# nirajbabar/raytracinginonesemester

Measured on AMD Instinct MI355X. Metric: Mrays/s at 1920x1080x16spp (1/2/4/8 GPU) + PPM max-abs pixel diff, higher is better.
Workload: dtype f32+f64

## Files before the change

### include/rt_mi355x.h

```cpp
#ifndef RT_MI355X_H
#define RT_MI355X_H

#include <stddef.h>
#include <stdint.h>

#ifdef __cplusplus
extern "C" {
#endif

#define RT_ABI_VERSION 3

enum {
    RT_OK = 0,
    RT_ERR_ARG = -1,
    RT_ERR_IO = -2,
    RT_ERR_PARSE = -3,
    RT_ERR_HIP = -4,
    RT_ERR_NOMEM = -5,
    RT_ERR_NODEVICE = -6,
    RT_ERR_UNSUPPORTED = -7,
    RT_ERR_COMM = -8,
    RT_ERR_INTERNAL = -9
};

// ... 142 lines not shown
int rt_render(rt_scene* s, const rt_camera* cam, const rt_render_opts* opt,
              float* rgb_host, int32_t* hit_idx_host, float* hit_t_host);

int rt_count_rays(rt_scene* s, const rt_camera* cam, const rt_render_opts* opt, uint64_t counts[3]);
int rt_count_rays_ex(rt_scene* s, const rt_camera* cam, const rt_render_opts* opt, uint64_t counts[4]);

int rt_render_reference(size_t num_triangles, int W, int H, const rt_camera* cam, rt_vec3 miss_color,
                        int max_depth, int spp, const rt_bvh_node* nodes, const rt_aabb* aabbs,
                        const rt_triangle* triangles, const int32_t* tri_object_ids,
                        const rt_material* materials, int num_materials, const rt_light* lights,
                        int num_lights, int diffuse_bounce, rt_vec3* output);

int rt_render_reference_gpus(size_t num_triangles, int W, int H, const rt_camera* cam, rt_vec3 miss_color,
                             int max_depth, int spp, const rt_bvh_node* nodes, const rt_aabb* aabbs,
                             const rt_triangle* triangles, const int32_t* tri_object_ids,
                             const rt_material* materials, int num_materials, const rt_light* lights,
                             int num_lights, int diffuse_bounce, int n_gpus, rt_vec3* output);

typedef struct rt_renderer rt_renderer;

enum {
    RT_DELIVER_P6 = 0,
    RT_DELIVER_F32 = 1,
    RT_DELIVER_DEVICE = 2,
    RT_DELIVER_NONE = 3
};
enum {
    RT_GATHER_AUTO = 0,
    RT_GATHER_RCCL = 1,
    RT_GATHER_DIRECT = 2,
    RT_GATHER_HOST_SHARED = 3
};
enum { RT_RENDERER_SELF_SEND = 1  };

typedef struct {
    int32_t n_devices;
    const int32_t* devices;
    int32_t world_size;
    int32_t rank0;
    const void* unique_id;
    int32_t band_rows;
    int32_t deliver;
    int32_t gather;
    int32_t depth;
    int32_t flags;
    const char* host_frame_name;
} rt_renderer_opts;
void rt_renderer_opts_default(rt_renderer_opts* o);

int rt_renderer_copy_engine(const rt_renderer* r);

int rt_comm_unique_id(void* id128);

int rt_renderer_create(size_t num_triangles, const rt_bvh_node* nodes, const rt_aabb* aabbs,
                       const rt_triangle* triangles, const int32_t* tri_object_ids,
                       const rt_material* materials, int num_materials, const rt_light* lights,
                       int num_lights, const rt_renderer_opts* opts, rt_renderer** out);
void rt_renderer_destroy(rt_renderer* r);

int rt_renderer_submit(rt_renderer* r, const rt_camera* cam, const rt_render_opts* opts, uint64_t* ticket);
int rt_renderer_submit_pair(rt_renderer* r, const rt_camera* cam_a, const rt_camera* cam_b,
                            const rt_render_opts* opts, uint64_t* ticket_a);
int rt_renderer_wait(rt_renderer* r, uint64_t ticket, const void** frame, size_t* bytes);
int rt_renderer_render(rt_renderer* r, const rt_camera* cam, const rt_render_opts* opts, void* out, size_t cap);
rt_scene* rt_renderer_scene(rt_renderer* r, int i);
int rt_renderer_local_ranks(const rt_renderer* r);
enum { RT_TIME_GATHER = 0, RT_TIME_DELIVER = 1, RT_TIME_FRAME = 2  };
int rt_renderer_times(rt_renderer* r, int kind, float* ms_out, int max, int* n_out);

int rt_render_hw1(int device, const rt_vec3* positions, const rt_vec3* normals,
                  const uint32_t* indices, size_t num_triangles, const rt_camera* cam,
                  rt_vec3 light_position, rt_vec3 light_color, int spp, const float* jitter,
                  float* rgb_host, int32_t* hit_idx_host, float* hit_t_host);

enum { RT_HW1_BRUTE = 1 };
int rt_render_hw1_ex(int device, const rt_vec3* positions, const rt_vec3* normals,
                     const uint32_t* indices, size_t num_triangles, const rt_camera* cam,
                     rt_vec3 light_position, rt_vec3 light_color, int spp, const float* jitter,
                     int flags, float* rgb_host, int32_t* hit_idx_host, float* hit_t_host,
                     float* kernel_ms);

typedef struct rt_hw1_scene rt_hw1_scene;
int rt_hw1_scene_create(int device, const rt_vec3* positions, const rt_vec3* normals, const uint32_t* indices,
                        size_t num_triangles, rt_hw1_scene** out);
void rt_hw1_scene_destroy(rt_hw1_scene* s);
int rt_render_hw1_device(rt_hw1_scene* s, const rt_camera* cam, rt_vec3 light_position, rt_vec3 light_color,
                         int spp, const float* jitter, int flags, float* rgb_dev, uint8_t* p6_dev,
                         int32_t* hit_idx_dev, float* hit_t_dev, void* hip_stream);
int rt_render_hw1_deliver(rt_hw1_scene* s, const rt_camera* cam, rt_vec3 light_position, rt_vec3 light_color,
                          int spp, int flags, uint8_t* host_p6, void* hip_stream, uint64_t* ticket);
int rt_hw1_wait(rt_hw1_scene* s, uint64_t ticket);
int rt_hw1_kernel_times(const rt_hw1_scene* s, float* ms_out, int max, int* n_out);
const char* rt_hw1_kernel_name(const rt_hw1_scene* s);
int rt_hw1_list_info(const rt_hw1_scene* s, int64_t info[2]);

int rt_intersect_rays(int device, const rt_triangle* tri, const float origin[3], const float* dirs, int n,
                      int hw1, float tmin, float tmax, int32_t* hit, float* t);

typedef struct { rt_vec3 origin, direction; } rt_ray;
enum { RT_RAYS_CLOSEST = 0, RT_RAYS_OCCLUDED = 1 };
enum { RT_RAYS_VARIANT_NONE = 0, RT_RAYS_VARIANT_WIDE = 1, RT_RAYS_VARIANT_BINARY = 2, RT_RAYS_VARIANT_DEEP = 3 };

int rt_trace_rays_device(rt_scene* s, int mode, const rt_ray* rays_dev, const float* max_t_dev, size_t n,
                         int flags, int32_t* hit_idx_dev, float* hit_t_dev, void* hip_stream);
int rt_trace_rays(rt_scene* s, int mode, const rt_ray* rays, const float* max_t, size_t n, int flags,
                  int32_t* hit_idx, float* hit_t, float* kernel_ms);
int rt_trace_rays_variant(const rt_scene* s);

float rt_powf_host(float x, float y);
int rt_powf_batch(int device, const float* x, const float* y, int n, float* out);

int rt_box_test_host(const float* rays, const float* boxes, const float* tminmax, int n,
                     int32_t* out_fast, int32_t* out_exact, int32_t* out_class);

int rt_debug_frustum_records(size_t P, const rt_bvh_node* nodes, const rt_aabb* aabbs, int max_log2, int stack_cap,
                             int64_t* info, float* rec, size_t rec_cap);

int rt_kernel_times(const rt_scene* s, float* ms_out, int max, int* n_out);
int rt_frame_times(const rt_scene* s, float* ms_out, int max, int* n_out);
int rt_prepass_times(const rt_scene* s, float* ms_out, int max, int* n_out);
int rt_live_tiles(const rt_scene* s, int64_t* live, int64_t* total);
int rt_heavy_tiles(const rt_scene* s, int64_t* heavy);
const char* rt_scene_kernel_name(const rt_scene* s);

int rt_scene_traversal_info(const rt_scene* s, int64_t info[4]);
int rt_scene_faults(rt_scene* s, uint32_t* flags, int clear);

typedef enum {
    RT_TUNE_FRUSTUM_ARITY = 0,
    RT_TUNE_HALF_WAVES = 1,
    RT_TUNE_PAIRED_ONLY = 2,
    RT_TUNE_HEAVY_FRAC = 3,
    RT_TUNE_HEAVY_CAP = 4,
    RT_TUNE_CULL_COVERAGE = 5,
    RT_TUNE_CULL_BOXES = 6,
    RT_TUNE_BIG_SCENE_BYTES = 7,
    RT_TUNE_FRUSTUM_STACK_CAP = 8,
    RT_TUNE_PEER_TIMEOUT_S = 9,
    RT_TUNE_RENDERER_THREADS = 10,
    RT_TUNE_COPY_ENGINE = 11,
    RT_TUNE_QUANT_RECORDS = 12,
    RT_TUNE_PREPASS_GATE = 13,
    RT_TUNE_OVERLAP_FRAMES = 14,
    RT_TUNE_KERNEL_TIMING_EVERY = 15,
    RT_TUNE_RECORD_GREEDY = 16,
    RT_TUNE_WIDE4_GREEDY = 17,
    RT_TUNE_PAIR_FRAMES = 18,
    RT_TUNE_PAIR_RESERVE = 19,
    RT_TUNE_CUT_SUB = 20,
    RT_TUNE_HW1_LANES = 21,
    RT_TUNE_COPY_WAIT = 22,
    RT_TUNE_HW1_FUSE = 23,
    RT_TUNE_HW1_CHUNK = 24,
    RT_TUNE_COUNT = 25
} rt_tune_id;
int rt_tuning_set(int id, double value);
int rt_tuning_get(int id, double* value);
void rt_tuning_reset(void);

int rt_device_count(int* n);
const char* rt_last_error(void);
int rt_abi_version(void);
const char* rt_build_id(void);

#ifdef __cplusplus
}
#endif
#endif
```

### raytracinginonesemester_amd/_lib.py

```python
from __future__ import annotations

import ctypes as C
import os
from pathlib import Path

PKG = Path(__file__).resolve().parent
LIB_PATH = Path(os.environ.get("RT_MI355X_LIB", PKG / "lib" / "librt_mi355x.so"))

RT_OK = 0
RT_ERR = {
    -1: "RT_ERR_ARG", -2: "RT_ERR_IO", -3: "RT_ERR_PARSE", -4: "RT_ERR_HIP",
    -5: "RT_ERR_NOMEM", -6: "RT_ERR_NODEVICE", -7: "RT_ERR_UNSUPPORTED", -8: "RT_ERR_COMM",
    -9: "RT_ERR_INTERNAL",
}
RT_KERNEL_AUTO, RT_KERNEL_WAVE, RT_KERNEL_LANE, RT_KERNEL_WAVE_PIXELS = 0, 1, 2, 3
RT_TILES_AUTO, RT_TILES_LINEAR, RT_TILES_XCD_CHUNK, RT_TILES_ROWS = 0, 1, 2, 3
RT_FLAG_NO_CULL = 1
RT_FLAG_BINARY = 4
RT_DELIVER_P6, RT_DELIVER_F32, RT_DELIVER_DEVICE, RT_DELIVER_NONE = 0, 1, 2, 3
RT_GATHER_AUTO, RT_GATHER_RCCL, RT_GATHER_DIRECT, RT_GATHER_HOST_SHARED = 0, 1, 2, 3
RT_RENDERER_SELF_SEND = 1
RT_TIME_GATHER, RT_TIME_DELIVER, RT_TIME_FRAME = 0, 1, 2
RT_FAULT_FRUSTUM_STACK = 1
RT_RAYS_CLOSEST, RT_RAYS_OCCLUDED = 0, 1
RT_RAYS_VARIANT_NONE, RT_RAYS_VARIANT_WIDE, RT_RAYS_VARIANT_BINARY, RT_RAYS_VARIANT_DEEP = 0, 1, 2, 3
TUNE = {"frustum_arity": 0, "half_waves": 1, "paired_only": 2, "heavy_frac": 3, "heavy_cap": 4,
        "cull_coverage": 5, "cull_boxes": 6, "big_scene_bytes": 7, "frustum_stack_cap": 8,
        "peer_timeout_s": 9, "renderer_threads": 10, "copy_engine": 11,
        "quant_records": 12, "prepass_gate": 13,
        "overlap_frames": 14, "kernel_timing_every": 15,
        "record_greedy": 16, "wide4_greedy": 17, "pair_frames": 18, "pair_reserve": 19,
        "cut_sub": 20, "hw1_lanes": 21, "copy_wait": 22, "hw1_fuse": 23, "hw1_chunk": 24}


class RTError(RuntimeError):
    def __init__(self, code: int, msg: str):
        super().__init__(f"{RT_ERR.get(code, code)}: {msg}")
        self.code = code


class Vec3(C.Structure):
    _fields_ = [("x", C.c_float), ("y", C.c_float), ("z", C.c_float)]

    def __iter__(self):
        return iter((self.x, self.y, self.z))


class BVHNode(C.Structure):
    _fields_ = [("parent_idx", C.c_uint32), ("left_idx", C.c_uint32),
                ("right_idx", C.c_uint32), ("object_idx", C.c_uint32)]


class AABB(C.Structure):
    _fields_ = [("min_corner", Vec3), ("max_corner", Vec3)]


class Triangle(C.Structure):
    _fields_ = [("v0", Vec3), ("v1", Vec3), ("v2", Vec3), ("n0", Vec3), ("n1", Vec3), ("n2", Vec3)]


class Material(C.Structure):
    _fields_ = [("albedo", Vec3), ("kd", C.c_float), ("specular_color", Vec3), ("ks", C.c_float),
                ("shininess", C.c_float), ("kr", C.c_float), ("emission", Vec3)]


class Light(C.Structure):
    _fields_ = [("position", Vec3), ("color", Vec3), ("intensity", C.c_int32)]


class CameraT(C.Structure):
    _fields_ = [("center", Vec3), ("pixel00_loc", Vec3), ("pixel_delta_u", Vec3),
                ("pixel_delta_v", Vec3), ("pixel_width", C.c_int32), ("pixel_height", C.c_int32)]


class SceneInfo(C.Structure):
    _fields_ = [("max_depth", C.c_int32), ("spp", C.c_int32), ("diffuse_bounce", C.c_int32),
                ("miss_color", Vec3), ("cam_position", Vec3), ("cam_look_at", Vec3), ("cam_up", Vec3),
                ("focal_length_mm", C.c_double), ("sensor_height_mm", C.c_double),
                ("pixel_width", C.c_int32), ("pixel_height", C.c_int32),
                ("num_triangles", C.c_uint64), ("num_vertices", C.c_uint64),
                ("num_materials", C.c_int32), ("num_lights", C.c_int32),
                ("num_objects_loaded", C.c_int32), ("bvh_max_stack", C.c_int32),
                ("bvh_height", C.c_int32)]


class SceneArrays(C.Structure):
    _fields_ = [("nodes", C.c_void_p), ("aabbs", C.c_void_p), ("triangles", C.c_void_p),
                ("tri_object_ids", C.c_void_p), ("materials", C.c_void_p), ("lights", C.c_void_p),
                ("positions", C.c_void_p), ("normals", C.c_void_p), ("indices", C.c_void_p)]


class MeshView(C.Structure):
    _fields_ = [("positions", C.c_void_p), ("normals", C.c_void_p), ("indices", C.c_void_p),
                ("num_vertices", C.c_uint64), ("num_triangles", C.c_uint64),
                ("has_normals", C.c_int32), ("has_uvs", C.c_int32)]


class PPMOptions(C.Structure):
    _fields_ = [("maxval", C.c_int32), ("clamp", C.c_int32), ("gamma2", C.c_int32), ("flip_y", C.c_int32)]


class RenderOpts(C.Structure):
    _fields_ = [("max_depth", C.c_int32), ("spp", C.c_int32), ("diffuse_bounce", C.c_int32),
                ("miss_color", Vec3), ("jitter", C.c_void_p), ("band_rows", C.c_int32),
                ("band_index", C.c_int32), ("band_count", C.c_int32), ("kernel", C.c_int32),
                ("tile_order", C.c_int32), ("flags", C.c_int32)]


class RendererOpts(C.Structure):
    _fields_ = [("n_devices", C.c_int32), ("devices", C.c_void_p), ("world_size", C.c_int32),
                ("rank0", C.c_int32), ("unique_id", C.c_void_p), ("band_rows", C.c_int32),
                ("deliver", C.c_int32), ("gather", C.c_int32), ("depth", C.c_int32), ("flags", C.c_int32),
                ("host_frame_name", C.c_void_p)]


P = C.c_void_p
I = C.c_int
SZ = C.c_size_t

SIGNATURES = {
    "rt_material_default": (None, [P]),
    "rt_camera_init": (I, [P, P, P, P, C.c_double, C.c_double, I, I, I]),
    "rt_jittered_samples": (I, [I, C.c_uint32, I, P]),
    "rt_host_scene_load_json": (I, [C.c_char_p, C.c_char_p, P]),
    "rt_host_scene_load_objs": (I, [P, I, P]),
    "rt_host_scene_info": (I, [P, P]),
    "rt_host_scene_arrays": (I, [P, P]),
    "rt_host_scene_free": (None, [P]),
    "rt_build_bvh": (I, [P, SZ, P, SZ, P, P]),
    "rt_build_bvh_device": (I, [I, P, SZ, P, SZ, P, P, P]),
    "rt_mesh_load_obj_hw1": (I, [C.c_char_p, P]),
    "rt_mesh_view_get": (I, [P, P]),
    "rt_mesh_free": (None, [P]),
    "rt_ppm_options_default": (None, [P]),
    "rt_ppm_write": (I, [C.c_char_p, P, I, I, P]),
    "rt_ppm_encode": (I, [P, I, I, P, P, SZ, P]),
    "rt_ppm_read": (I, [C.c_char_p, P, SZ, P, P, P]),
    "rt_ppm_header": (I, [I, I, I, P, SZ, P]),
    "rt_ppm_quantize_device": (I, [P, I, I, P, P, P]),
    "rt_unpermute_strips_device": (I, [P, I, SZ, I, I, I, I, P, P]),
    "rt_scene_create": (I, [I, SZ, P, P, P, P, P, I, P, I, P]),
    "rt_scene_destroy": (None, [P]),
    "rt_scene_clone": (I, [P, I, P]),
    "rt_scene_device": (I, [P]),
    "rt_scene_device_bytes": (SZ, [P]),
    "rt_render_opts_default": (None, [P]),
    "rt_shard_rows": (I, [I, I, I, I]),
    "rt_render_device": (I, [P, P, P, P, P, P, P]),
    "rt_render_device_p6": (I, [P, P, P, P, P, P, P, P]),
    "rt_render_device_pair": (I, [P, P, P, P, P, P, P, P, P]),
    "rt_render": (I, [P, P, P, P, P, P]),
    "rt_count_rays": (I, [P, P, P, P]),
    "rt_count_rays_ex": (I, [P, P, P, P]),
    "rt_render_reference": (I, [SZ, I, I, P, Vec3, I, I, P, P, P, P, P, I, P, I, I, P]),
    "rt_render_reference_gpus": (I, [SZ, I, I, P, Vec3, I, I, P, P, P, P, P, I, P, I, I, I, P]),
    "rt_renderer_opts_default": (None, [P]),
    "rt_comm_unique_id": (I, [P]),
    "rt_renderer_create": (I, [SZ, P, P, P, P, P, I, P, I, P, P]),
    "rt_renderer_destroy": (None, [P]),
    "rt_renderer_submit": (I, [P, P, P, P]),
    "rt_renderer_submit_pair": (I, [P, P, P, P, P]),
    "rt_renderer_wait": (I, [P, C.c_uint64, P, P]),
    "rt_renderer_render": (I, [P, P, P, P, SZ]),
    "rt_renderer_scene": (P, [P, I]),
    "rt_renderer_local_ranks": (I, [P]),
    "rt_renderer_copy_engine": (I, [P]),
    "rt_renderer_times": (I, [P, I, P, I, P]),
    "rt_render_hw1": (I, [I, P, P, P, SZ, P, Vec3, Vec3, I, P, P, P, P]),
    "rt_render_hw1_ex": (I, [I, P, P, P, SZ, P, Vec3, Vec3, I, P, I, P, P, P, P]),
    "rt_hw1_scene_create": (I, [I, P, P, P, SZ, P]),
    "rt_hw1_scene_destroy": (None, [P]),
    "rt_render_hw1_device": (I, [P, P, Vec3, Vec3, I, P, I, P, P, P, P, P]),
    "rt_render_hw1_deliver": (I, [P, P, Vec3, Vec3, I, I, P, P, P]),
    "rt_hw1_wait": (I, [P, C.c_uint64]),
    "rt_hw1_kernel_times": (I, [P, P, I, P]),
    "rt_hw1_kernel_name": (C.c_char_p, [P]),
    "rt_hw1_list_info": (I, [P, P]),
    "rt_intersect_rays": (I, [I, P, P, P, I, I, C.c_float, C.c_float, P, P]),
    "rt_trace_rays_device": (I, [P, I, P, P, SZ, I, P, P, P]),
    "rt_trace_rays": (I, [P, I, P, P, SZ, I, P, P, P]),
    "rt_trace_rays_variant": (I, [P]),
    "rt_powf_host": (C.c_float, [C.c_float, C.c_float]),
    "rt_debug_frustum_records": (C.c_int, [C.c_size_t, P, P, C.c_int, C.c_int, P, P, C.c_size_t]),
    "rt_powf_batch": (I, [I, P, P, I, P]),
    "rt_box_test_host": (I, [P, P, P, I, P, P, P]),
# ... 53 lines not shown
```

### raytracinginonesemester_amd/csrc/rt_device.hip

```cpp

#include <hip/hip_runtime.h>
#include <hip/hip_ext.h>

#include <cfloat>
#include <cmath>
#include <cstdint>
#include <cstdio>
#include <cstdlib>
#include <cstring>
#include <algorithm>
#include <atomic>
#include <functional>
#include <memory>
#include <new>
#include <string>
#include <array>
#include <vector>

#include "rt_common.hpp"
#include "rt_hip_host.hpp"
#include "rt_math.hpp"
#include "rt_ppm.hpp"
#include "rt_records.hpp"

// ... 1017 lines not shown
        if (hipOccupancyMaxActiveBlocksPerMultiprocessor(&n, KERNEL, BLOCK, 0) != hipSuccess || n < 1) n = 1;
        return n;
    }();
    static const std::string name = "render_tiles_kernel<" + std::to_string(MODE) + (SAMPLES ? ", true" : ", false") +
                                    (D1 ? ", true, " : ", false, ") + std::to_string(WAVES) + ", " +
                                    std::to_string(LS) + ">";
    if (L.name) *L.name = name.c_str();
    const int tiles8 = (P.tiles_total + 7) / 8 * 8;
    const dim3 grid((unsigned)std::max(8, std::min(tiles8, L.cus * per_cu / 8 * 8)));
    hipExtLaunchKernelGGL(KERNEL, grid, dim3(BLOCK), 0, L.st, L.start, L.stop, 0, P);
}

template <int MODE, bool SAMPLES, bool D1, int WAVES = RT_RENDER_WAVES, int LS = 0>
void launch_render_pair(const RenderParams& A, const RenderParams& B, const Launch& L, double reserve_default) {
    constexpr auto KERNEL = render_pair_kernel<MODE, SAMPLES, D1, WAVES, LS>;
    static const int per_cu = [] {
        int n = 0;
        if (hipOccupancyMaxActiveBlocksPerMultiprocessor(&n, KERNEL, BLOCK, 0) != hipSuccess || n < 1) n = 1;
        return n;
    }();
    static const std::string name = "render_pair_kernel<" + std::to_string(MODE) + (SAMPLES ? ", true" : ", false") +
                                    (D1 ? ", true, " : ", false, ") + std::to_string(WAVES) + ", " +
                                    std::to_string(LS) + ">";
    if (L.name) *L.name = name.c_str();
    const int tiles8 = (A.tiles_total + B.tiles_total + 7) / 8 * 8;
    const double reserve = std::clamp(rt::tuning(RT_TUNE_PAIR_RESERVE, reserve_default), 0.0, double(per_cu - 1));
    const int blocks = L.cus * per_cu - int(std::lround(reserve * L.cus));
    const dim3 grid((unsigned)std::max(8, std::min(tiles8, blocks / 8 * 8)));
    PairParams PP;
    PP.f[0] = A;
    PP.f[1] = B;
    hipExtLaunchKernelGGL(KERNEL, grid, dim3(BLOCK), 0, L.st, L.start, L.stop, 0, PP);
}

bool pair_kernel_fits(const RenderParams& P, bool samples, bool wave_wide, bool big) {
    const bool d1 = P.max_depth == 1;
    const bool bounce = P.max_depth > 1 && P.half_waves && P.paired_only;
    return samples && wave_wide && !big && (d1 || bounce) && P.nqueues == 8 && P.spp <= 64 && !P.ray_count &&
           P.lane_samples == 1;
}
void launch_pair(const RenderParams& A, const RenderParams& B, const Launch& L) {
    constexpr int M = RT_KERNEL_WAVE | MODE_WIDE | MODE_PK;
    if (A.max_depth > 1) launch_render_pair<RT_KERNEL_WAVE | MODE_WIDE, true, false, RT_PAIRED_WAVES, 3>(A, B, L, 0.0);
    else if (A.half_waves) launch_render_pair<M, true, true, RT_RENDER_WAVES, 1>(A, B, L, 1.0);
    else launch_render_pair<M, true, true>(A, B, L, 1.0);
}

template <int MODE, bool SAMPLES>
void launch_mode(const RenderParams& P, const Launch& L) {
    constexpr int D1_MODE = (MODE & (MODE_DEEP | RT_KERNEL_LANE)) == 0 ? (MODE | MODE_PK) : MODE;
    if (P.max_depth == 1) {
        if constexpr (SAMPLES) {
            if (P.half_waves) {
                launch_render<D1_MODE, SAMPLES, true, RT_RENDER_WAVES, 1>(P, L);
                return;
            }
        }
        if constexpr ((MODE & (MODE_DEEP | RT_KERNEL_LANE)) == 0) {
            if (L.big) {
                if constexpr ((MODE & MODE_WIDE) != 0) {
                    if (L.qr) {
                        if (P.sc.num_lights == 1)
                            launch_render<D1_MODE | MODE_1L | MODE_QR, SAMPLES, true, RT_RENDER_WAVES_BIG>(P, L);
                        else launch_render<D1_MODE | MODE_QR, SAMPLES, true, RT_RENDER_WAVES_BIG>(P, L);
                        return;
                    }
                }
                if (P.sc.num_lights == 1) launch_render<D1_MODE | MODE_1L, SAMPLES, true, RT_RENDER_WAVES_BIG>(P, L);
                else launch_render<D1_MODE, SAMPLES, true, RT_RENDER_WAVES_BIG>(P, L);
                return;
            }
        }
        launch_render<D1_MODE, SAMPLES, true>(P, L);
    } else {
        if constexpr (SAMPLES && (MODE & (MODE_DEEP | RT_KERNEL_LANE)) == 0) {
            if (P.half_waves && P.paired_only) {
                launch_render<MODE, SAMPLES, false, RT_PAIRED_WAVES, 3>(P, L);
                return;
            }
        }
        if constexpr (SAMPLES) {
            if (P.half_waves) {
                launch_render<MODE, SAMPLES, false, RT_BOUNCE_WAVES, 1>(P, L);
                return;
            }
        }
        launch_render<MODE, SAMPLES, false, RT_BOUNCE_WAVES>(P, L);
    }
}

template <int MODE>
void launch(const RenderParams& P, bool samples, const Launch& L) {
    if (samples) launch_mode<MODE, true>(P, L);
    else launch_mode<MODE, false>(P, L);
}

f3 miss_pixel_value(const rt_render_opts* o) {
    f3 c = mk(0.f, 0.f, 0.f);
    if (o->max_depth > 0)
        c = clamp01(add(mk(0.f, 0.f, 0.f), mul(mk(1.f, 1.f, 1.f), f3{o->miss_color.x, o->miss_color.y, o->miss_color.z})));
    f3 acc = mk(0.f, 0.f, 0.f);
    for (int k = 0; k < o->spp; ++k) acc = add(acc, c);
    const float fs = (float)o->spp;
    return f3{acc.x / fs, acc.y / fs, acc.z / fs};
}

}

namespace {
double root_box_coverage(const float* rb, const rt_camera* cam) {
    const double c[3] = {cam->center.x, cam->center.y, cam->center.z};
    const double b0[3] = {cam->pixel00_loc.x - c[0], cam->pixel00_loc.y - c[1], cam->pixel00_loc.z - c[2]};
    const double du[3] = {cam->pixel_delta_u.x, cam->pixel_delta_u.y, cam->pixel_delta_u.z};
    const double dv[3] = {cam->pixel_delta_v.x, cam->pixel_delta_v.y, cam->pixel_delta_v.z};
    auto det3 = [](const double* x, const double* y, const double* z) {
        return x[0] * (y[1] * z[2] - y[2] * z[1]) - y[0] * (x[1] * z[2] - x[2] * z[1]) + z[0] * (x[1] * y[2] - x[2] * y[1]);
    };
    const double D = det3(b0, du, dv);
    if (!(std::fabs(D) > 0.0) || !(rb[0] <= rb[3] && rb[1] <= rb[4] && rb[2] <= rb[5])) return 1.0;
    double x0 = INFINITY, x1 = -INFINITY, y0 = INFINITY, y1 = -INFINITY;
    for (int k = 0; k < 8; ++k) {
        const double p[3] = {double(rb[(k & 1) ? 3 : 0]) - c[0], double(rb[(k & 2) ? 4 : 1]) - c[1],
                             double(rb[(k & 4) ? 5 : 2]) - c[2]};
        const double sx = det3(p, du, dv) / D, a = det3(b0, p, dv) / D, b = det3(b0, du, p) / D;
        if (!(sx > 0.0)) return 1.0;
        x0 = std::min(x0, a / sx);
        x1 = std::max(x1, a / sx);
        y0 = std::min(y0, b / sx);
        y1 = std::max(y1, b / sx);
    }
    const double W = cam->pixel_width, H = cam->pixel_height;
    const double w = std::max(0.0, std::min(W, x1) - std::max(0.0, x0)), h = std::max(0.0, std::min(H, y1) - std::max(0.0, y0));
    return w * h / (W * H);
}
}

thread_local unsigned long long* t_ray_count = nullptr;

extern "C" int rt_render_device(rt_scene* s, const rt_camera* cam, const rt_render_opts* o, float* rgb,
                                int32_t* hit_idx, float* hit_t, void* stream) {
    return rt_render_device_p6(s, cam, o, rgb, hit_idx, hit_t, nullptr, stream);
}

namespace {
struct PairStage {
    int phase = 0;
    bool deferred = false;
    RenderParams A;
    Launch LA{};
    uint64_t kA = 0;
    hipStream_t stream = nullptr;
};

int launch_prepasses(rt_scene* s, const RenderParams& P, int slot) {
    const bool cut = P.cull && P.sc.ncut > 0;
    hipExtLaunchKernelGGL(tile_cull_kernel, dim3((P.tiles_total + BLOCK - 1) / BLOCK), dim3(BLOCK), 0, s->prep,
                          s->ev0[slot], cut ? nullptr : s->pdone[slot], 0, P);
    HIP_TRY(hipGetLastError());
    if (cut) {
        const int cut_blocks = 4 * s->cus;
        hipExtLaunchKernelGGL(tile_cut_kernel, dim3(cut_blocks), dim3(BLOCK), 0, s->prep, nullptr, s->pdone[slot], 0, P);
        HIP_TRY(hipGetLastError());
    }
    return RT_OK;
}

int flush_pair_a(rt_scene* s, PairStage& ps) {
    if (!ps.deferred) return RT_OK;
    ps.deferred = false;
    const int slot = int(ps.kA % rt_scene::kRing);
    s->span[slot] = 1;
    if (int rc = launch_prepasses(s, ps.A, slot); rc != RT_OK) return rc;
    HIP_TRY(hipStreamWaitEvent(ps.LA.st, s->pdone[slot], 0));
    launch<RT_KERNEL_WAVE | MODE_WIDE>(ps.A, true, ps.LA);
    HIP_TRY(hipGetLastError());
    if (ps.A.drained) s->drain_frame = ps.kA;
    return RT_OK;
}

int render_frame(rt_scene* s, const rt_camera* cam, const rt_render_opts* o, float* rgb, int32_t* hit_idx,
                 float* hit_t, uint8_t* p6, void* stream, PairStage* ps);
}

extern "C" int rt_render_device_p6(rt_scene* s, const rt_camera* cam, const rt_render_opts* o, float* rgb,
                                   int32_t* hit_idx, float* hit_t, uint8_t* p6, void* stream) {
    return render_frame(s, cam, o, rgb, hit_idx, hit_t, p6, stream, nullptr);
}

extern "C" int rt_render_device_pair(rt_scene* s, const rt_camera* cam_a, const rt_camera* cam_b,
                                     const rt_render_opts* o, float* rgb_a, uint8_t* p6_a, float* rgb_b,
                                     uint8_t* p6_b, void* stream) {
    if (!s || !cam_a || !cam_b || !o || (!rgb_a && !p6_a) || (!rgb_b && !p6_b))
        return set_error(RT_ERR_ARG, "rt_render_device_pair: null argument");
    PairStage ps;
    int rc = render_frame(s, cam_a, o, rgb_a, nullptr, nullptr, p6_a, stream, &ps);
    if (rc != RT_OK) return rc;
    ps.phase = 1;
    rc = render_frame(s, cam_b, o, rgb_b, nullptr, nullptr, p6_b, stream, &ps);
    if (ps.deferred) {
        DeviceGuard g(s->device);
        const int rc2 = flush_pair_a(s, ps);
        if (rc == RT_OK) rc = rc2;
    }
    return rc;
}

namespace {
int render_frame(rt_scene* s, const rt_camera* cam, const rt_render_opts* o, float* rgb, int32_t* hit_idx,
                 float* hit_t, uint8_t* p6, void* stream, PairStage* ps) {
    if (!s || !cam || !o || (!rgb && !p6)) return set_error(RT_ERR_ARG, "rt_render_device: null argument");
    if (o->spp < 1) return set_error(RT_ERR_ARG, "spp must be >= 1");
    if ((hit_idx == nullptr) != (hit_t == nullptr)) return set_error(RT_ERR_ARG, "hit_idx and hit_t go together");
    const int W = cam->pixel_width, H = cam->pixel_height;
    if (W < 1 || H < 1) return set_error(RT_ERR_ARG, "camera has no pixels");
    const int rows = rt_shard_rows(H, o->band_rows, o->band_index, o->band_count);
    if (rows < 0) return set_error(RT_ERR_ARG, "bad band sharding parameters");
    DeviceGuard g(s->device);
    int rc = prepare_jitter(s, o);
    if (rc != RT_OK) return rc;
    if (rows == 0) return RT_OK;

    RenderParams P;
    std::memset(&P, 0, sizeof(P));
    P.sc.inode = static_cast<const float4*>(s->inode.p);
    P.sc.wnode = static_cast<const float4*>(s->wnode.p);
    P.sc.fnode = static_cast<const float*>(s->fnode.p);
    P.sc.f_log2 = s->fnode.p ? s->f_log2 : 2;
    P.sc.qent = static_cast<const uint4*>(s->qent.p);
    P.sc.qhdr = static_cast<const float4*>(s->qhdr.p);
    P.sc.wide = s->wide && !(o->flags & RT_FLAG_BINARY) ? 1 : 0;
    P.sc.lane_stack = s->lane_stack ? 1 : 0;
    P.sc.lane_wide = s->lane_wide ? 1 : 0;
    P.sc.ibox = static_cast<const float4*>(s->ibox.p);
    P.sc.rootb = static_cast<const float4*>(s->ibox.p) + s->ibox.n / sizeof(float4) - 2;
    P.sc.leaf = static_cast<const float4*>(s->leaf.p);
    P.sc.tnorm = static_cast<const float4*>(s->tnorm.p);
    P.sc.objids = static_cast<const int32_t*>(s->objids.p);
    P.sc.mats = static_cast<const DevMaterial*>(s->mats.p);
    P.sc.lights = static_cast<const DevLight*>(s->lights.p);
    P.sc.num_tris = int32_t(s->P);
    P.sc.num_mats = s->nmat;
    P.sc.num_lights = s->nlights;
    P.sc.root_ref = s->root_ref;
    std::memcpy(P.sc.root_box, s->root_box, sizeof(P.sc.root_box));
    P.sc.cut = static_cast<const float*>(s->cut.p);
    P.sc.cut2 = static_cast<const float*>(s->cut2.p);
    P.sc.cut_sub_log2 = s->cut2.p ? s->cut_sub_log2 : 0;
    P.sc.tri = static_cast<const float4*>(s->tri.p);
    P.sc.fault = static_cast<uint32_t*>(s->fault.p);
    const double max_cov = rt::tuning(RT_TUNE_CULL_COVERAGE, 0.3);
    P.sc.ncut = s->ncut > 0 && root_box_coverage(s->root_box, cam) <= max_cov ? s->ncut : 0;
    P.cut_force = max_cov >= 1.0 ? 1 : 0;
    std::memcpy(P.sc.bmax, s->bmax, sizeof(P.sc.bmax));
    P.cam_center = f3{cam->center.x, cam->center.y, cam->center.z};
    P.cam_p00 = f3{cam->pixel00_loc.x, cam->pixel00_loc.y, cam->pixel00_loc.z};
    P.cam_du = f3{cam->pixel_delta_u.x, cam->pixel_delta_u.y, cam->pixel_delta_u.z};
    P.cam_dv = f3{cam->pixel_delta_v.x, cam->pixel_delta_v.y, cam->pixel_delta_v.z};
    P.W = W;
    P.H = H;
    P.spp = o->spp;
    P.max_depth = o->max_depth;
    P.diffuse_bounce = o->diffuse_bounce ? 1 : 0;
    P.miss = f3{o->miss_color.x, o->miss_color.y, o->miss_color.z};
    P.jitter = static_cast<const float*>(s->jitter.p);
    P.band_rows = o->band_count <= 1 ? H : o->band_rows;
    P.band_index = o->band_count <= 1 ? 0 : o->band_index;
    P.band_count = o->band_count <= 1 ? 1 : o->band_count;
    P.rows = rows;
    P.rgb = rgb;
    P.hit_idx = hit_idx;
    P.hit_t = hit_t;
    P.p6 = p6;
    P.ray_count = t_ray_count;
    {
        const f3 mp = miss_pixel_value(o);
        P.miss_p6[0] = rtp::p6_default_sample(mp.x);
        P.miss_p6[1] = rtp::p6_default_sample(mp.y);
        P.miss_p6[2] = rtp::p6_default_sample(mp.z);
        P.miss_p6[3] = 0;
    }
    const bool samples = o->kernel != RT_KERNEL_WAVE_PIXELS && o->spp <= BLOCK && (o->spp & (o->spp - 1)) == 0;
    int half = o->band_count >= 4 || o->max_depth > 1 ? 1 : 0;
    if (const double h = rt::tuning(RT_TUNE_HALF_WAVES, -1.0); h >= 0.0) half = h >= 1.0 ? 1 : 0;
    if (!samples || o->spp > (64 >> half)) half = 0;
    P.half_waves = half;
    P.paired_only = half && o->max_depth > 1 && s->nlights == 1 && !s->deep && o->kernel != RT_KERNEL_LANE &&
                            (P.sc.wide ? s->lane_wide : s->lane_stack)
                        ? 1
                        : 0;
    P.paired_only = P.paired_only && rt::tuning(RT_TUNE_PAIRED_ONLY, 1.0) != 0.0;
    int ppb = samples ? (BLOCK >> half) / o->spp : BLOCK;
    int tw = 1;
    while (tw * tw < ppb) tw <<= 1;
    int th = ppb / tw;
    P.tile_w = tw;
    P.tile_h = th;
    P.tile_w_log2 = __builtin_ctz(unsigned(tw));
    P.spp_log2 = samples ? __builtin_ctz(unsigned(o->spp)) : 0;
    P.tiles_x = (W + tw - 1) / tw;
    const int tiles_y = (rows + th - 1) / th;
    P.tiles_total = P.tiles_x * tiles_y;
    P.lane_samples = samples ? 1 : 0;
    P.tile_order = o->tile_order == RT_TILES_AUTO ? RT_TILES_ROWS : o->tile_order;
    P.cull = (o->flags & RT_FLAG_NO_CULL) ? 0 : 1;
    if (!P.cull) P.sc.ncut = 0;
    P.miss_pixel = miss_pixel_value(o);
    P.nqueues = P.tile_order == RT_TILES_LINEAR ? 1 : 8;
    P.queue_cap = P.tile_order == RT_TILES_LINEAR ? P.tiles_total : P.tiles_x * ((tiles_y + 7) / 8);
// ... 602 lines not shown
```

### raytracinginonesemester_amd/csrc/rt_prepass.hpp

```cpp
#pragma once

struct TileDirs {
    double c[3], Dl[3], Dh[3], iDl[3], iDh[3], scale;
    bool usable;
};
__device__ __forceinline__ TileDirs tile_dirs(const RenderParams& P, int x0, int x1, int y0, int y1) {
    TileDirs T;
    const double p0[3] = {P.cam_p00.x, P.cam_p00.y, P.cam_p00.z};
    const double du[3] = {P.cam_du.x, P.cam_du.y, P.cam_du.z};
    const double dv[3] = {P.cam_dv.x, P.cam_dv.y, P.cam_dv.z};
    T.c[0] = P.cam_center.x;
    T.c[1] = P.cam_center.y;
    T.c[2] = P.cam_center.z;
    const double pxl = x0 - 1.0, pxh = x1 + 1.0, pyl = y0 - 1.0, pyh = y1 + 1.0;
    const double pxm = fmax(fabs(pxl), fabs(pxh)), pym = fmax(fabs(pyl), fabs(pyh));
    T.scale = 0.0;
#pragma unroll
    for (int a = 0; a < 3; ++a) {
        const double base = p0[a] - T.c[a];
        const double u0 = pxl * du[a], u1 = pxh * du[a], v0 = pyl * dv[a], v1 = pyh * dv[a];
        const double ulp = 8.0 * 1.1920928955078125e-7 * (fabs(T.c[a]) + fabs(p0[a]) + pxm * fabs(du[a]) + pym * fabs(dv[a]));
        T.Dl[a] = base + fmin(u0, u1) + fmin(v0, v1) - ulp;
        T.Dh[a] = base + fmax(u0, u1) + fmax(v0, v1) + ulp;
        T.scale = fmax(T.scale, fmax(fabs(T.Dl[a]), fabs(T.Dh[a])));
// ... 109 lines not shown
}

__device__ __forceinline__ int global_row(const RenderParams& P, int r) {
    if (P.band_count <= 1) return r;
    const int k = r / P.band_rows, within = r - k * P.band_rows;
    return (P.band_index + k * P.band_count) * P.band_rows + within;
}

constexpr int COUNTER_STRIDE = 64;
#ifndef RT_NCLASS
#define RT_NCLASS 5
#endif
constexpr int NCLASS = RT_NCLASS;
constexpr int NCLASS_D1 = 3;
constexpr int HEAVY_SLOT0 = 9;
constexpr int CUT_SLOT0 = HEAVY_SLOT0 + 8 * NCLASS;
constexpr int HEAD_SLOT0 = CUT_SLOT0 + 8;
constexpr int COUNTER_SLOTS = HEAD_SLOT0 + 8;
constexpr int COUNTER_SET_U32 = COUNTER_SLOTS * COUNTER_STRIDE;
__host__ __device__ constexpr int heavy_counter(int k, int q) { return (HEAVY_SLOT0 + 8 * k + q) * COUNTER_STRIDE; }
__device__ __forceinline__ int queue_of_tile(const RenderParams& P, int tile) {
    if (P.nqueues == 1) return 0;
    if (P.tile_order == RT_TILES_XCD_CHUNK) return (int)((int64_t)tile * 8 / P.tiles_total);
    return (tile / P.tiles_x) & 7;
}

__device__ __forceinline__ void write_culled_tile(const RenderParams& P, int tile, int first, int lanes) {
    const int tx = tile % P.tiles_x, ty = tile / P.tiles_x;
    const int xa = tx * P.tile_w, ra = ty * P.tile_h;
    const int tw = min(xa + P.tile_w, P.W) - xa, th = min(ra + P.tile_h, P.rows) - ra;
    const float mp[3] = {P.miss_pixel.x, P.miss_pixel.y, P.miss_pixel.z};
    if (lanes == 1 && tw == 4 && (xa & 3) == 0 && (P.W & 3) == 0 && ((uintptr_t)P.rgb & 15) == 0 &&
        ((uintptr_t)P.p6 & 3) == 0) {
        const float4 f0 = make_float4(mp[0], mp[1], mp[2], mp[0]), f1 = make_float4(mp[1], mp[2], mp[0], mp[1]),
                     f2 = make_float4(mp[2], mp[0], mp[1], mp[2]);
        const uint32_t b0 = P.miss_p6[0], b1 = P.miss_p6[1], b2 = P.miss_p6[2];
        const uint32_t w0 = b0 | b1 << 8 | b2 << 16 | b0 << 24, w1 = b1 | b2 << 8 | b0 << 16 | b1 << 24,
                       w2 = b2 | b0 << 8 | b1 << 16 | b2 << 24;
        for (int r = ra; r < ra + th; ++r) {
            if (P.rgb) {
                float4* o = reinterpret_cast<float4*>(P.rgb + ((size_t)r * P.W + xa) * 3);
                o[0] = f0;
                o[1] = f1;
                o[2] = f2;
            }
            if (P.p6) {
                uint32_t* q = reinterpret_cast<uint32_t*>(P.p6 + ((size_t)r * P.W + xa) * 3);
                q[0] = w0;
                q[1] = w1;
                q[2] = w2;
            }
        }
    } else {
        for (int i = first; i < tw * th * 3; i += lanes) {
            const int px = i / 3, c = i - 3 * px;
            const int r = ra + px / tw, x = xa + px % tw;
            if (P.rgb) P.rgb[((size_t)r * P.W + x) * 3 + c] = c == 0 ? mp[0] : c == 1 ? mp[1] : mp[2];
            if (P.p6) P.p6[((size_t)r * P.W + x) * 3 + c] = c == 0 ? P.miss_p6[0] : c == 1 ? P.miss_p6[1] : P.miss_p6[2];
        }
    }
    if (P.hit_idx) {
        for (int i = first; i < tw * th * P.spp; i += lanes) {
            const int px = i / P.spp, smp = i - P.spp * px;
            const int r = ra + px / tw, x = xa + px % tw;
            const size_t k = ((size_t)r * P.W + x) * (size_t)P.spp + smp;
            P.hit_idx[k] = -1;
            P.hit_t[k] = -1.0f;
        }
    }
}

__device__ __forceinline__ void append_live(const RenderParams& P, bool live, int tile) {
    const int q = live ? queue_of_tile(P, tile) : 0;
    const uint32_t lane = lane_id();
    uint64_t pending = ballot(live);
    while (pending != 0) {
        const uint32_t leader = (uint32_t)__builtin_ctzll(pending);
        const int lq = rdlane(q, leader);
        const uint64_t m = pending & ballot(q == lq);
        uint32_t base = 0;
        if (lane == leader) base = atomicAdd(&P.live_count[lq * COUNTER_STRIDE], (uint32_t)__popcll(m));
        base = rdlane(base, leader);
        if ((m >> lane) & 1ull)
            P.live_tiles[(size_t)lq * P.queue_cap + base + (uint32_t)__popcll(m & ((1ull << lane) - 1))] = tile;
        pending &= ~m;
    }
}

__device__ __forceinline__ void cull_tiles(const RenderParams& P, int tile) {
    bool live = false;
    if (tile < P.tiles_total) {
        const int tx = tile % P.tiles_x, ty = tile / P.tiles_x;
        const int xa = tx * P.tile_w, ra = ty * P.tile_h;
        const int xb = min(xa + P.tile_w, P.W) - 1, rb = min(ra + P.tile_h, P.rows) - 1;
        const bool culled = P.cull && tile_misses_root(P, xa, xb, global_row(P, ra), global_row(P, rb));
        if (culled) write_culled_tile(P, tile, 0, 1);
        else live = true;
    }
    append_live(P, live, tile);
}

__global__ __launch_bounds__(BLOCK) void tile_cull_kernel(RenderParams P) {
    __builtin_amdgcn_s_setprio(3);
    if (blockIdx.x == 0 && threadIdx.x < COUNTER_SLOTS) P.next_count[threadIdx.x * COUNTER_STRIDE] = 0u;
#ifdef RT_FRAME_SPAN
    if (threadIdx.x == 0 && g_frame_span) atomicMin(&g_frame_span[4 * (P.drain_tag & 255u) + 2], wall_clock64());
#endif
    cull_tiles(P, (int)(blockIdx.x * BLOCK + threadIdx.x));
}

#ifndef RT_CUT_GROUP
#define RT_CUT_GROUP 8
#endif
constexpr int CUT_GROUP = RT_CUT_GROUP;
__device__ __forceinline__ bool cut_setup(const RenderParams& P, uint32_t lane, float* box, int& max_len) {
    int n = 0;
    max_len = 0;
    for (int k = 0; k < P.nqueues; ++k) {
        const int l = (int)ldc_u32(&P.live_count[k * COUNTER_STRIDE]);
        n += l;
        max_len = max(max_len, l);
    }
    const bool test = P.cut_force || 4 * (int64_t)n <= (int64_t)P.tiles_total;
    if (test && (int)lane < P.sc.ncut) {
#pragma unroll
        for (int i = 0; i < 6; ++i) box[i] = P.sc.cut[6 * (size_t)lane + i];
    }
    return test;
}

__device__ __forceinline__ bool tile_cut_sub(const RenderParams& P, const TileDirsF& T, uint64_t hm, uint32_t lane) {
    const int sl = P.sc.cut_sub_log2;
    const int per = 64 >> sl;
    const int gi = (int)(lane >> sl);
    const uint32_t c = lane & ((1u << sl) - 1u);
    while (hm != 0) {
        int mine = -1;
        for (int k = 0; k < per && hm != 0; ++k) {
            const int b = __builtin_ctzll(hm);
            if (gi == k) mine = b;
            hm &= hm - 1;
        }
        bool reach = false;
        if (mine >= 0) {
            const float* p = P.sc.cut2 + 6 * (((size_t)mine << sl) | c);
            const float bx[6] = {p[0], p[1], p[2], p[3], p[4], p[5]};
            reach = !tile_misses_box_f(T, bx);
        }
        if (ballot(reach) != 0) return true;
    }
    return false;
}

__device__ __forceinline__ bool cut_unit(const RenderParams& P, uint32_t lane, int q, int g, bool test,
                                         const float* box) {
    const int len = (int)ldc_u32(&P.live_count[q * COUNTER_STRIDE]);
    if (CUT_GROUP * g >= len) return false;
    const int m = min(CUT_GROUP, len - CUT_GROUP * g);
    const size_t slot0 = (size_t)q * P.queue_cap + (size_t)(CUT_GROUP * g);
    const int my_tile = (int)lane < m ? P.live_tiles[slot0 + lane] : -1;
    uint2 cost = make_uint2(0u, 0u);
    if (P.heavy_cap > 0 && (int)lane < m) cost = *reinterpret_cast<const uint2*>(P.tile_cost + 4 * (size_t)my_tile);
    uint64_t culled = 0;
    for (int j = 0; test && j < m; ++j) {
        const int tile = (int)rdlane((uint32_t)my_tile, (uint32_t)j);
        const int tx = tile % P.tiles_x, ty = tile / P.tiles_x;
        const int xa = tx * P.tile_w, ra = ty * P.tile_h;
        const int xb = min(xa + P.tile_w, P.W) - 1, rb = min(ra + P.tile_h, P.rows) - 1;
        const TileDirsF T = tile_dirs_f(P, xa, xb, global_row(P, ra), global_row(P, rb));
        const bool hit = (int)lane < P.sc.ncut && !tile_misses_box_f(T, box);
#ifdef RT_WAVE_TIMES
        {
            const uint64_t hm = ballot(hit);
            if (g_cut_counts && lane == 0) g_cut_counts[tile] = __popcll(hm);
        }
#endif
        const uint64_t hm = ballot(hit);
        if (hm == 0 || (P.sc.cut_sub_log2 > 0 && !tile_cut_sub(P, T, hm, lane))) {
            write_culled_tile(P, tile, (int)lane, 64);
            culled |= 1ull << j;
        }
    }
    int cls = -1;
    if ((int)lane < m && !((culled >> lane) & 1ull)) {
        cls = NCLASS;
        if (P.heavy_cap > 0) {
            const uint32_t mx = max(max(cost.x & 0xffffu, cost.x >> 16), max(cost.y & 0xffffu, cost.y >> 16));
            for (int k = NCLASS - 1; k >= 0; --k)
                if (mx >= P.heavy_ticks[k]) cls = k;
        }
    }
    uint64_t cm[NCLASS + 1];
    uint32_t add = 0;
#pragma unroll
    for (int k = 0; k <= NCLASS; ++k) {
        cm[k] = ballot(cls == k);
        if ((int)lane == k) add = (uint32_t)__popcll(cm[k]);
    }
    const uint64_t below = (1ull << lane) - 1;
    if (ballot(add != 0) != 0) {
        uint32_t base = 0;
        if ((int)lane <= NCLASS && add != 0)
            base = atomicAdd(&P.live_count[(int)lane < NCLASS ? heavy_counter((int)lane, q) : (CUT_SLOT0 + q) * COUNTER_STRIDE], add);
        bool spill = false;
#pragma unroll
        for (int k = 0; k <= NCLASS; ++k) {
            const uint32_t idx = rdlane(base, (uint32_t)k) + (uint32_t)__popcll(cm[k] & below);
            if (cls == k) {
                if (k == NCLASS) P.cut_tiles[(size_t)q * P.queue_cap + idx] = my_tile;
                else if (idx < (uint32_t)P.heavy_cap) P.heavy_tiles[((size_t)k * 8 + q) * P.heavy_cap + idx] = my_tile;
                else spill = true;
            }
        }
        const uint64_t sm = ballot(spill);
        if (sm != 0) {
            const uint32_t leader = (uint32_t)__builtin_ctzll(sm);
            uint32_t b2 = 0;
            if (lane == leader) b2 = atomicAdd(&P.live_count[(CUT_SLOT0 + q) * COUNTER_STRIDE], (uint32_t)__popcll(sm));
            if (spill) P.cut_tiles[(size_t)q * P.queue_cap + rdlane(b2, leader) + (uint32_t)__popcll(sm & below)] = my_tile;
        }
    }
    return true;
}

__global__ __launch_bounds__(BLOCK) void tile_cut_kernel(RenderParams P) {
    __builtin_amdgcn_s_setprio(3);
    const uint32_t lane = lane_id();
    const int waves = (int)(gridDim.x * (BLOCK / 64));
    float box[6] = {0.f, 0.f, 0.f, -1.f, -1.f, -1.f};
    int max_len;
    const bool test = cut_setup(P, lane, box, max_len);
    for (int p = (int)(blockIdx.x * (BLOCK / 64) + threadIdx.x / 64);; p += waves) {
        const int q = p % P.nqueues, g = p / P.nqueues;
        if (CUT_GROUP * g >= max_len) break;
        (void)cut_unit(P, lane, q, g, test, box);
    }
#ifdef RT_FRAME_SPAN
    if (lane == 0 && g_frame_span) atomicMax(&g_frame_span[4 * (P.drain_tag & 255u) + 3], wall_clock64());
#endif
}
```

Baseline: 230,500.

## Add fused tile cull+cut prepass kernel behind tuning knob

Adds a single tile_prepass_kernel that runs the root-box cull and the per-cut-box culling in one pass over contiguous tile runs, appending survivors straight into per-queue class lists instead of launching tile_cull_kernel followed by tile_cut_kernel. It also refactors cut_unit so each lane computes its own tile directions once and broadcasts them via readlane, instead of recomputing them per iteration. The fused path is gated by a new RT_TUNE_PREPASS_FUSED knob whose default is 0, so by default only the readlane refactor of cut_unit runs. The fused kernel changes how queue counters are incremented and may alter the order of tile lists.

```diff
diff --git a/include/rt_mi355x.h b/include/rt_mi355x.h
--- a/include/rt_mi355x.h
+++ b/include/rt_mi355x.h
@@ -318,7 +318,8 @@
     RT_TUNE_COPY_WAIT = 22,
     RT_TUNE_HW1_FUSE = 23,
     RT_TUNE_HW1_CHUNK = 24,
-    RT_TUNE_COUNT = 25
+    RT_TUNE_PREPASS_FUSED = 25,
+    RT_TUNE_COUNT = 26
 } rt_tune_id;
 int rt_tuning_set(int id, double value);
 int rt_tuning_get(int id, double* value);
diff --git a/raytracinginonesemester_amd/_lib.py b/raytracinginonesemester_amd/_lib.py
--- a/raytracinginonesemester_amd/_lib.py
+++ b/raytracinginonesemester_amd/_lib.py
@@ -30,7 +30,8 @@
         "quant_records": 12, "prepass_gate": 13,
         "overlap_frames": 14, "kernel_timing_every": 15,
         "record_greedy": 16, "wide4_greedy": 17, "pair_frames": 18, "pair_reserve": 19,
-        "cut_sub": 20, "hw1_lanes": 21, "copy_wait": 22, "hw1_fuse": 23, "hw1_chunk": 24}
+        "cut_sub": 20, "hw1_lanes": 21, "copy_wait": 22, "hw1_fuse": 23, "hw1_chunk": 24,
+        "prepass_fused": 25}
 
 
 class RTError(RuntimeError):
diff --git a/raytracinginonesemester_amd/csrc/rt_device.hip b/raytracinginonesemester_amd/csrc/rt_device.hip
--- a/raytracinginonesemester_amd/csrc/rt_device.hip
+++ b/raytracinginonesemester_amd/csrc/rt_device.hip
@@ -1193,8 +1193,19 @@
     hipStream_t stream = nullptr;
 };
 
+constexpr int kPrepassFusedRun = 0;
+
 int launch_prepasses(rt_scene* s, const RenderParams& P, int slot) {
     const bool cut = P.cull && P.sc.ncut > 0;
+    const int run = int(std::clamp(rt::tuning(RT_TUNE_PREPASS_FUSED, double(kPrepassFusedRun)), 0.0, 64.0));
+    if (cut && run > 0) {
+        const int units = (P.tiles_total + run - 1) / run;
+        const int blocks = std::min(4 * s->cus, (units + BLOCK / 64 - 1) / (BLOCK / 64));
+        hipExtLaunchKernelGGL(tile_prepass_kernel, dim3(blocks), dim3(BLOCK), 0, s->prep, s->ev0[slot], s->pdone[slot], 0,
+                              P, run);
+        HIP_TRY(hipGetLastError());
+        return RT_OK;
+    }
     hipExtLaunchKernelGGL(tile_cull_kernel, dim3((P.tiles_total + BLOCK - 1) / BLOCK), dim3(BLOCK), 0, s->prep,
                           s->ev0[slot], cut ? nullptr : s->pdone[slot], 0, P);
     HIP_TRY(hipGetLastError());
diff --git a/raytracinginonesemester_amd/csrc/rt_prepass.hpp b/raytracinginonesemester_amd/csrc/rt_prepass.hpp
--- a/raytracinginonesemester_amd/csrc/rt_prepass.hpp
+++ b/raytracinginonesemester_amd/csrc/rt_prepass.hpp
@@ -285,6 +285,87 @@
     return false;
 }
 
+__device__ __forceinline__ int tile_class(const RenderParams& P, uint2 cost) {
+    int cls = NCLASS;
+    if (P.heavy_cap > 0) {
+        const uint32_t mx = max(max(cost.x & 0xffffu, cost.x >> 16), max(cost.y & 0xffffu, cost.y >> 16));
+        for (int k = NCLASS - 1; k >= 0; --k)
+            if (mx >= P.heavy_ticks[k]) cls = k;
+    }
+    return cls;
+}
+
+__device__ __forceinline__ void append_classed(const RenderParams& P, uint32_t lane, int q, int cls, int my_tile,
+                                               uint32_t roots) {
+    uint64_t cm[NCLASS + 1];
+    uint32_t add = (int)lane == NCLASS + 1 ? roots : 0u;
+#pragma unroll
+    for (int k = 0; k <= NCLASS; ++k) {
+        cm[k] = ballot(cls == k);
+        if ((int)lane == k) add = (uint32_t)__popcll(cm[k]);
+    }
+    const uint64_t below = (1ull << lane) - 1;
+    if (ballot(add != 0) != 0) {
+        uint32_t base = 0;
+        if ((int)lane <= NCLASS + 1 && add != 0)
+            base = atomicAdd(&P.live_count[(int)lane < NCLASS    ? heavy_counter((int)lane, q)
+                                           : (int)lane == NCLASS ? (CUT_SLOT0 + q) * COUNTER_STRIDE
+                                                                 : q * COUNTER_STRIDE],
+                             add);
+        bool spill = false;
+#pragma unroll
+        for (int k = 0; k <= NCLASS; ++k) {
+            const uint32_t idx = rdlane(base, (uint32_t)k) + (uint32_t)__popcll(cm[k] & below);
+            if (cls == k) {
+                if (k == NCLASS) P.cut_tiles[(size_t)q * P.queue_cap + idx] = my_tile;
+                else if (idx < (uint32_t)P.heavy_cap) P.heavy_tiles[((size_t)k * 8 + q) * P.heavy_cap + idx] = my_tile;
+                else spill = true;
+            }
+        }
+        const uint64_t sm = ballot(spill);
+        if (sm != 0) {
+            const uint32_t leader = (uint32_t)__builtin_ctzll(sm);
+            uint32_t b2 = 0;
+            if (lane == leader) b2 = atomicAdd(&P.live_count[(CUT_SLOT0 + q) * COUNTER_STRIDE], (uint32_t)__popcll(sm));
+            if (spill) P.cut_tiles[(size_t)q * P.queue_cap + rdlane(b2, leader) + (uint32_t)__popcll(sm & below)] = my_tile;
+        }
+    }
+}
+
+__device__ __forceinline__ TileDirsF tile_dirs_of(const RenderParams& P, int tile) {
+    const int tx = tile % P.tiles_x, ty = tile / P.tiles_x;
+    const int xa = tx * P.tile_w, ra = ty * P.tile_h;
+    const int xb = min(xa + P.tile_w, P.W) - 1, rb = min(ra + P.tile_h, P.rows) - 1;
+    return tile_dirs_f(P, xa, xb, global_row(P, ra), global_row(P, rb));
+}
+__device__ __forceinline__ float rdlane_f(float v, uint32_t l) { return __uint_as_float(rdlane(__float_as_uint(v), l)); }
+__device__ __forceinline__ TileDirsF tile_dirs_from_lane(const TileDirsF& M, uint32_t j) {
+    TileDirsF T;
+#pragma unroll
+    for (int a = 0; a < 3; ++a) {
+        T.c[a] = rdlane_f(M.c[a], j);
+        T.Dl[a] = rdlane_f(M.Dl[a], j);
+        T.Dh[a] = rdlane_f(M.Dh[a], j);
+        T.iDl[a] = rdlane_f(M.iDl[a], j);
+        T.iDh[a] = rdlane_f(M.iDh[a], j);
+    }
+    T.scale = rdlane_f(M.scale, j);
+    T.usable = rdlane(M.usable ? 1u : 0u, j) != 0;
+    return T;
+}
+
+__device__ __forceinline__ bool tile_cut_culls(const RenderParams& P, uint32_t lane, int tile, const TileDirsF& T,
+                                               const float* box) {
+    const bool hit = (int)lane < P.sc.ncut && !tile_misses_box_f(T, box);
+    const uint64_t hm = ballot(hit);
+#ifdef RT_WAVE_TIMES
+    if (g_cut_counts && lane == 0) g_cut_counts[tile] = __popcll(hm);
+#endif
+    if (hm != 0 && (P.sc.cut_sub_log2 <= 0 || tile_cut_sub(P, T, hm, lane))) return false;
+    write_culled_tile(P, tile, (int)lane, 64);
+    return true;
+}
+
 __device__ __forceinline__ bool cut_unit(const RenderParams& P, uint32_t lane, int q, int g, bool test,
                                          const float* box) {
     const int len = (int)ldc_u32(&P.live_count[q * COUNTER_STRIDE]);
@@ -295,64 +376,13 @@
     uint2 cost = make_uint2(0u, 0u);
     if (P.heavy_cap > 0 && (int)lane < m) cost = *reinterpret_cast<const uint2*>(P.tile_cost + 4 * (size_t)my_tile);
     uint64_t culled = 0;
-    for (int j = 0; test && j < m; ++j) {
-        const int tile = (int)rdlane((uint32_t)my_tile, (uint32_t)j);
-        const int tx = tile % P.tiles_x, ty = tile / P.tiles_x;
-        const int xa = tx * P.tile_w, ra = ty * P.tile_h;
-        const int xb = min(xa + P.tile_w, P.W) - 1, rb = min(ra + P.tile_h, P.rows) - 1;
-        const TileDirsF T = tile_dirs_f(P, xa, xb, global_row(P, ra), global_row(P, rb));
-        const bool hit = (int)lane < P.sc.ncut && !tile_misses_box_f(T, box);
-#ifdef RT_WAVE_TIMES
-        {
-            const uint64_t hm = ballot(hit);
-            if (g_cut_counts && lane == 0) g_cut_counts[tile] = __popcll(hm);
-        }
-#endif
-        const uint64_t hm = ballot(hit);
-        if (hm == 0 || (P.sc.cut_sub_log2 > 0 && !tile_cut_sub(P, T, hm, lane))) {
-            write_culled_tile(P, tile, (int)lane, 64);
+    const TileDirsF mine = tile_dirs_of(P, max(my_tile, 0));
+    for (int j = 0; test && j < m; ++j)
+        if (tile_cut_culls(P, lane, (int)rdlane((uint32_t)my_tile, (uint32_t)j), tile_dirs_from_lane(mine, (uint32_t)j), box))
             culled |= 1ull << j;
-        }
-    }
     int cls = -1;
-    if ((int)lane < m && !((culled >> lane) & 1ull)) {
-        cls = NCLASS;
-        if (P.heavy_cap > 0) {
-            const uint32_t mx = max(max(cost.x & 0xffffu, cost.x >> 16), max(cost.y & 0xffffu, cost.y >> 16));
-            for (int k = NCLASS - 1; k >= 0; --k)
-                if (mx >= P.heavy_ticks[k]) cls = k;
-        }
-    }
-    uint64_t cm[NCLASS + 1];
-    uint32_t add = 0;
-#pragma unroll
-    for (int k = 0; k <= NCLASS; ++k) {
-        cm[k] = ballot(cls == k);
-        if ((int)lane == k) add = (uint32_t)__popcll(cm[k]);
-    }
-    const uint64_t below = (1ull << lane) - 1;
-    if (ballot(add != 0) != 0) {
-        uint32_t base = 0;
-        if ((int)lane <= NCLASS && add != 0)
-            base = atomicAdd(&P.live_count[(int)lane < NCLASS ? heavy_counter((int)lane, q) : (CUT_SLOT0 + q) * COUNTER_STRIDE], add);
-        bool spill = false;
-#pragma unroll
-        for (int k = 0; k <= NCLASS; ++k) {
-            const uint32_t idx = rdlane(base, (uint32_t)k) + (uint32_t)__popcll(cm[k] & below);
-            if (cls == k) {
-                if (k == NCLASS) P.cut_tiles[(size_t)q * P.queue_cap + idx] = my_tile;
-                else if (idx < (uint32_t)P.heavy_cap) P.heavy_tiles[((size_t)k * 8 + q) * P.heavy_cap + idx] = my_tile;
-                else spill = true;
-            }
-        }
-        const uint64_t sm = ballot(spill);
-        if (sm != 0) {
-            const uint32_t leader = (uint32_t)__builtin_ctzll(sm);
-            uint32_t b2 = 0;
-            if (lane == leader) b2 = atomicAdd(&P.live_count[(CUT_SLOT0 + q) * COUNTER_STRIDE], (uint32_t)__popcll(sm));
-            if (spill) P.cut_tiles[(size_t)q * P.queue_cap + rdlane(b2, leader) + (uint32_t)__popcll(sm & below)] = my_tile;
-        }
-    }
+    if ((int)lane < m && !((culled >> lane) & 1ull)) cls = tile_class(P, cost);
+    append_classed(P, lane, q, cls, my_tile, 0u);
     return true;
 }
 
@@ -372,3 +402,51 @@
     if (lane == 0 && g_frame_span) atomicMax(&g_frame_span[4 * (P.drain_tag & 255u) + 3], wall_clock64());
 #endif
 }
+
+__device__ __forceinline__ void prepass_unit(const RenderParams& P, uint32_t lane, int unit, int run, const float* box) {
+    const int tile0 = unit * run;
+    const int m = min(run, P.tiles_total - tile0);
+    const int my_tile = (int)lane < m ? tile0 + (int)lane : -1;
+    uint2 cost = make_uint2(0u, 0u);
+    if (P.heavy_cap > 0 && my_tile >= 0) cost = *reinterpret_cast<const uint2*>(P.tile_cost + 4 * (size_t)my_tile);
+    const TileDirsF mine = tile_dirs_of(P, max(my_tile, 0));
+    bool live = false;
+    if (my_tile >= 0) {
+        if (tile_misses_box_f(mine, P.sc.root_box)) write_culled_tile(P, my_tile, 0, 1);
+        else live = true;
+    }
+    const uint64_t roots = ballot(live);
+    uint64_t kept = roots;
+    for (uint64_t r = roots; r != 0; r &= r - 1) {
+        const int j = __builtin_ctzll(r);
+        if (tile_cut_culls(P, lane, tile0 + j, tile_dirs_from_lane(mine, (uint32_t)j), box)) kept &= ~(1ull << j);
+    }
+    const int cls = (kept >> lane) & 1ull ? tile_class(P, cost) : -1;
+    const int q = live ? queue_of_tile(P, my_tile) : 0;
+    for (uint64_t pending = roots; pending != 0;) {
+        const int lq = (int)rdlane((uint32_t)q, (uint32_t)__builtin_ctzll(pending));
+        const uint64_t qm = pending & ballot(q == lq);
+        append_classed(P, lane, lq, (qm >> lane) & 1ull ? cls : -1, my_tile, (uint32_t)__popcll(qm));
+        pending &= ~qm;
+    }
+}
+
+__global__ __launch_bounds__(BLOCK) void tile_prepass_kernel(RenderParams P, int run) {
+    __builtin_amdgcn_s_setprio(3);
+    if (blockIdx.x == 0 && threadIdx.x < COUNTER_SLOTS) P.next_count[threadIdx.x * COUNTER_STRIDE] = 0u;
+#ifdef RT_FRAME_SPAN
+    if (threadIdx.x == 0 && g_frame_span) atomicMin(&g_frame_span[4 * (P.drain_tag & 255u) + 2], wall_clock64());
+#endif
+    const uint32_t lane = lane_id();
+    float box[6] = {0.f, 0.f, 0.f, -1.f, -1.f, -1.f};
+    if ((int)lane < P.sc.ncut) {
+#pragma unroll
+        for (int i = 0; i < 6; ++i) box[i] = P.sc.cut[6 * (size_t)lane + i];
+    }
+    const int units = (P.tiles_total + run - 1) / run;
+    const int waves = (int)(gridDim.x * (BLOCK / 64));
+    for (int u = (int)uni(blockIdx.x * (BLOCK / 64) + threadIdx.x / 64); u < units; u += waves) prepass_unit(P, lane, u, run, box);
+#ifdef RT_FRAME_SPAN
+    if (lane == 0 && g_frame_span) atomicMax(&g_frame_span[4 * (P.drain_tag & 255u) + 3], wall_clock64());
+#endif
+}
```

Result: no change. 230,700, median of 3 (+0.1%).
